# zeyadmohamedabdo/Visual-Question-Answering-VQA-system

Hardware: AMD Instinct MI355X
Metric: image-question pairs/sec (train step) (higher is better)
Workload: dtype bf16; 1 GPU; VQA train step fwd+CE+bwd+allreduce+clip+AdamW, batch 512/GPU, 3x224x224 images, 20 tokens, d=256, 4 text layers, 49 image tokens, 1000 answers, dropout on (BASELINE configs[2]); batch_per_gpu=512, global_batch=512, parallelism=dp1, reducer=off

## Files before the change

visual-question-answering-vqa-system_amd/csrc/cnn_ops.hip:

```cpp
#include "common.h"
#include "stem_route.h"

__global__ void bn_reduce_partials_kernel(const float* __restrict__ part, double* __restrict__ acc, int tiles, int C) {
  const int c = blockIdx.x * 64 + (threadIdx.x & 63), tl = threadIdx.x >> 6;
  __shared__ double sh[2][4][64];
  double s = 0.0, q = 0.0;
  if (c < C) {
    const int step = gridDim.y * 4;
    int t = blockIdx.y * 4 + tl;
    for (; t + 7 * step < tiles; t += 8 * step) {
      float a[8], b[8];
#pragma unroll
      for (int u = 0; u < 8; ++u) { a[u] = part[((size_t)(t + u * step) * 2) * C + c]; b[u] = part[((size_t)(t + u * step) * 2 + 1) * C + c]; }
#pragma unroll
      for (int u = 0; u < 8; ++u) { s += (double)a[u]; q += (double)b[u]; }
    }
    for (; t < tiles; t += step) {
      s += (double)part[((size_t)t * 2) * C + c];
      q += (double)part[((size_t)t * 2 + 1) * C + c];
    }
  }
  sh[0][tl][threadIdx.x & 63] = s; sh[1][tl][threadIdx.x & 63] = q;
  __syncthreads();
  if (tl == 0 && c < C) {
// ... 248 lines not shown
template <typename T, bool SELF, bool DUAL>
__global__ __launch_bounds__(256) void bn_bwd_apply_kernel(const T* __restrict__ dout, const T* __restrict__ outact, const T* __restrict__ y,
                                    const float* __restrict__ bc, T* __restrict__ dy, const T* __restrict__ y2,
                                    const float* __restrict__ bc2, T* __restrict__ dy2, size_t rows, int C,
                                    const float* __restrict__ mcoef) {
  constexpr int VEC = Vec16<T>::N;
  const int cv = C / VEC, lanes_r = 256 / cv;
  const int c0 = (threadIdx.x % cv) * VEC, myr = threadIdx.x / cv;
  float a[VEC], b[VEC], c[VEC], a2[DUAL ? VEC : 1], b2[DUAL ? VEC : 1], c2[DUAL ? VEC : 1], ms[SELF ? VEC : 1], mh[SELF ? VEC : 1];
#pragma unroll
  for (int j = 0; j < VEC; ++j) {
    a[j] = bc[c0 + j]; b[j] = bc[C + c0 + j]; c[j] = bc[2 * C + c0 + j];
    if (DUAL) { a2[j] = bc2[c0 + j]; b2[j] = bc2[C + c0 + j]; c2[j] = bc2[2 * C + c0 + j]; }
    if (SELF) { ms[j] = mcoef[c0 + j]; mh[j] = mcoef[C + c0 + j]; }
  }
#pragma unroll 2
  for (size_t r = (size_t)blockIdx.x * lanes_r + myr; r < rows; r += (size_t)gridDim.x * lanes_r) {
    const size_t off = r * C + c0;
    Vec16<T> d = ldg16(dout + off), yy = ldg16(y + off), o, y2v, rr, r2;
    if (!SELF && outact) o = ldg16(outact + off);
    if (DUAL) y2v = ldg16(y2 + off);
#pragma unroll
    for (int j = 0; j < VEC; ++j) {
      float g = d.get(j);
      if (SELF) { if (!(yy.get(j) * ms[j] + mh[j] > 0.f)) g = 0.f; }
      else if (outact && !(o.get(j) > 0.f)) g = 0.f;
      rr.set(j, a[j] * g + b[j] * yy.get(j) + c[j]);
      if (DUAL) r2.set(j, a2[j] * g + b2[j] * y2v.get(j) + c2[j]);
    }
    stg16(dy + off, rr);
    if (DUAL) stg16(dy2 + off, r2);
  }
}

template <typename T, bool SELF, bool DUAL>
__global__ __launch_bounds__(256) void bn_bwd_apply_acc_kernel(const T* __restrict__ dout, const T* __restrict__ outact, const T* __restrict__ y,
                                    const unsigned long long* __restrict__ facc, const float* __restrict__ gamma, const float* __restrict__ coef,
                                    float* dgamma, float* dbeta, T* __restrict__ dy, const T* __restrict__ y2, const float* __restrict__ gamma2,
                                    const float* __restrict__ coef2, float* dgamma2, float* dbeta2, T* __restrict__ dy2, size_t rows, int C,
                                    double inv_count) {
  constexpr int VEC = Vec16<T>::N;
  const int cv = C / VEC, lanes_r = 256 / cv;
  const int c0 = (threadIdx.x % cv) * VEC, myr = threadIdx.x / cv;
  const bool writer = blockIdx.x == 0;
  const int R = acc_replicas(C);
  const bool bad = acc_flagged(facc, R, 3, C);
  extern __shared__ float cf[];
  for (int ch = threadIdx.x; ch < C; ch += 256) {
    double sg = acc_read_fixed(facc, R, 3, C, 0, ch), sx = acc_read_fixed(facc, R, 3, C, 1, ch);
    if (bad) sg = sx = __builtin_nan("");
    const float mean = coef[2 * C + ch], invstd = coef[3 * C + ch], gi = gamma[ch] * invstd;
    const float mg = (float)(sg * inv_count), mgx = (float)(sx * inv_count);
    cf[ch] = gi; cf[C + ch] = -gi * invstd * mgx; cf[2 * C + ch] = gi * (mean * invstd * mgx - mg);
    if (writer) { dgamma[ch] += (float)sx; dbeta[ch] += (float)sg; }
    if (DUAL) {
      double sx2 = acc_read_fixed(facc, R, 3, C, 2, ch);
      if (bad) sx2 = __builtin_nan("");
      const float mean2 = coef2[2 * C + ch], inv2 = coef2[3 * C + ch], gi2 = gamma2[ch] * inv2, mgx2 = (float)(sx2 * inv_count);
      cf[3 * C + ch] = gi2; cf[4 * C + ch] = -gi2 * inv2 * mgx2; cf[5 * C + ch] = gi2 * (mean2 * inv2 * mgx2 - mg);
      if (writer) { dgamma2[ch] += (float)sx2; dbeta2[ch] += (float)sg; }
    }
  }
  __syncthreads();
  float a[VEC], b[VEC], c[VEC], a2[DUAL ? VEC : 1], b2[DUAL ? VEC : 1], c2[DUAL ? VEC : 1], ms[SELF ? VEC : 1], mh[SELF ? VEC : 1];
#pragma unroll
  for (int j = 0; j < VEC; ++j) {
    const int ch = c0 + j;
    a[j] = cf[ch]; b[j] = cf[C + ch]; c[j] = cf[2 * C + ch];
    if (DUAL) { a2[j] = cf[3 * C + ch]; b2[j] = cf[4 * C + ch]; c2[j] = cf[5 * C + ch]; }
    if (SELF) { ms[j] = coef[ch]; mh[j] = coef[C + ch]; }
  }
#pragma unroll 2
  for (size_t r = (size_t)blockIdx.x * lanes_r + myr; r < rows; r += (size_t)gridDim.x * lanes_r) {
    const size_t off = r * C + c0;
    Vec16<T> d = ldg16(dout + off), yy = ldg16(y + off), o, y2v, rr, r2;
    if (!SELF && outact) o = ldg16(outact + off);
    if (DUAL) y2v = ldg16(y2 + off);
#pragma unroll
    for (int j = 0; j < VEC; ++j) {
      float g = d.get(j);
      if (SELF) { if (!(yy.get(j) * ms[j] + mh[j] > 0.f)) g = 0.f; }
      else if (outact && !(o.get(j) > 0.f)) g = 0.f;
      rr.set(j, a[j] * g + b[j] * yy.get(j) + c[j]);
      if (DUAL) r2.set(j, a2[j] * g + b2[j] * y2v.get(j) + c2[j]);
    }
    stg16(dy + off, rr);
    if (DUAL) stg16(dy2 + off, r2);
  }
}

constexpr int SP_ROWS = 4, SP_PAIRS = 7;
template <typename T>
__global__ __launch_bounds__(256) void stem_pool_fwd_kernel(const T* __restrict__ y, const float* __restrict__ coef, T* __restrict__ out,
                                                            uint8_t* __restrict__ idx, int B, int H, int W, int C, int Ho, int Wo, int trows) {
  constexpr int VEC = Vec16<T>::N;
  const int cv = C / VEC, Wp = (Wo + 1) >> 1;
  const int tiles_x = (Wp + SP_PAIRS - 1) / SP_PAIRS, tiles_y = (Ho + trows - 1) / trows;
  const int per_row = SP_PAIRS * cv;
  const int ry = threadIdx.x / per_row, rem = threadIdx.x - ry * per_row;
  if (ry >= trows) return;
  const int pr = rem / cv, c0 = (rem - pr * cv) * VEC;
  int t = blockIdx.x;
  const int tx = t % tiles_x; t /= tiles_x; const int ty = t % tiles_y; const int b = t / tiles_y;
  const int oh = ty * trows + ry, owp = tx * SP_PAIRS + pr;
  if (oh >= Ho || owp >= Wp) return;
  float sc[VEC], sh[VEC];
#pragma unroll
  for (int j = 0; j < VEC; ++j) { sc[j] = coef[c0 + j]; sh[j] = coef[C + c0 + j]; }
  const int ow0 = owp * 2;
  const bool two = ow0 + 1 < Wo;
  float best[2][VEC]; int bi[2][VEC];
#pragma unroll
  for (int o = 0; o < 2; ++o)
#pragma unroll
    for (int j = 0; j < VEC; ++j) { best[o][j] = -INFINITY; bi[o][j] = 0; }
#pragma unroll
  for (int r = 0; r < 3; ++r) {
    const int ih = oh * 2 - 1 + r;
    if (ih < 0 || ih >= H) continue;
    const T* yr = y + (((size_t)b * H + ih) * W) * C + c0;
#pragma unroll
    for (int s5 = 0; s5 < 5; ++s5) {
      const int iw = ow0 * 2 - 1 + s5;
      if (iw < 0 || iw >= W) continue;
      const Vec16<T> yy = ldg16(yr + (size_t)iw * C);
      float a[VEC];
#pragma unroll
      for (int j = 0; j < VEC; ++j) { const float v = yy.get(j) * sc[j] + sh[j]; a[j] = v < 0.f ? 0.f : v; }
      if (s5 < 3) {
#pragma unroll
        for (int j = 0; j < VEC; ++j)
          if (a[j] > best[0][j] || a[j] != a[j]) { best[0][j] = a[j]; bi[0][j] = r * 3 + s5; }
      }
      if (s5 >= 2) {
#pragma unroll
        for (int j = 0; j < VEC; ++j)
          if (a[j] > best[1][j] || a[j] != a[j]) { best[1][j] = a[j]; bi[1][j] = r * 3 + s5 - 2; }
      }
    }
  }
#pragma unroll
  for (int o = 0; o < 2; ++o) {
    if (o == 1 && !two) break;
    const size_t e = ((((size_t)b * Ho + oh) * Wo + ow0 + o) * C + c0);
    Vec16<T> ov;
    uint32_t pk[VEC / 4];
#pragma unroll
    for (int q4 = 0; q4 < VEC / 4; ++q4) pk[q4] = 0u;
#pragma unroll
    for (int j = 0; j < VEC; ++j) { ov.set(j, best[o][j]); pk[j >> 2] |= (uint32_t)bi[o][j] << (8 * (j & 3)); }
    stg16(out + e, ov);
#pragma unroll
    for (int q4 = 0; q4 < VEC / 4; ++q4) reinterpret_cast<uint32_t*>(idx + e)[q4] = pk[q4];
  }
}

template <typename T>
__global__ void stem_bwd_apply_kernel(const T* __restrict__ dpool, const uint8_t* __restrict__ idx, const T* __restrict__ y,
                                      const float* __restrict__ coef, const float* __restrict__ bc, T* __restrict__ dy,
                                      int B, int H, int W, int C, int Ho, int Wo) {
  constexpr int VEC = Vec16<T>::N;
  const int cv = C / VEC;
  const size_t total = (size_t)B * H * W * cv;
  float g[VEC];
  for (size_t i = (size_t)blockIdx.x * blockDim.x + threadIdx.x; i < total; i += (size_t)gridDim.x * blockDim.x) {
    const int v = (int)(i % cv); size_t r = i / cv;
    const int w = (int)(r % W); size_t q = r / W; const int h = (int)(q % H); const int b = (int)(q / H);
    const int c0 = v * VEC;
    Vec16<T> yy = ldg16(y + i * VEC), o;
    float sc[VEC], sh[VEC];
#pragma unroll
    for (int j = 0; j < VEC; ++j) { sc[j] = coef[c0 + j]; sh[j] = coef[C + c0 + j]; }
    stem_route<T>(dpool, idx, yy, sc, sh, b, h, w, c0, C, Ho, Wo, g);
#pragma unroll
    for (int j = 0; j < VEC; ++j) o.set(j, bc[c0 + j] * g[j] + bc[C + c0 + j] * yy.get(j) + bc[2 * C + c0 + j]);
    stg16(dy + i * VEC, o);
  }
}

template <typename T>
__global__ __launch_bounds__(256) void se_pool_fc_kernel(const T* __restrict__ x, const float* __restrict__ w1, const float* __restrict__ w2,
                                                         float* __restrict__ pooled, float* __restrict__ hidden, float* __restrict__ scale,
                                                         int HW, int C, int Cr, const float* __restrict__ part, int chunks) {
  constexpr int VEC = Vec16<T>::N;
  extern __shared__ float sh[];
  const int b = blockIdx.x, cv = C / VEC, lanes_r = 256 / cv;
  const int myv = threadIdx.x % cv, myr = threadIdx.x / cv;
  float s[VEC];
#pragma unroll
  for (int j = 0; j < VEC; ++j) s[j] = 0.f;
  if (!part && myr < lanes_r) {
    const T* xb = x + (size_t)b * HW * C + myv * VEC;
    int p = myr;
    for (; p + 3 * lanes_r < HW; p += 4 * lanes_r) {
      Vec16<T> v0 = ldg16(xb + (size_t)p * C), v1 = ldg16(xb + (size_t)(p + lanes_r) * C);
      Vec16<T> v2 = ldg16(xb + (size_t)(p + 2 * lanes_r) * C), v3 = ldg16(xb + (size_t)(p + 3 * lanes_r) * C);
#pragma unroll
      for (int j = 0; j < VEC; ++j) s[j] += (v0.get(j) + v1.get(j)) + (v2.get(j) + v3.get(j));
    }
    for (; p < HW; p += lanes_r) {
      Vec16<T> v = ldg16(xb + (size_t)p * C);
#pragma unroll
      for (int j = 0; j < VEC; ++j) s[j] += v.get(j);
    }
  }
#pragma unroll
  for (int j = 0; j < VEC; ++j) sh[threadIdx.x * VEC + j] = s[j];
  __syncthreads();
  float* pl = sh + 256 * VEC; float* hd = pl + C;
  for (int c = threadIdx.x; c < C; c += 256) {
    const int v = c / VEC, j = c - v * VEC;
    float t = 0.f;
    if (part) { for (int k = 0; k < chunks; ++k) t += part[((size_t)b * chunks + k) * C + c]; }
    else { for (int r = 0; r < lanes_r; ++r) t += sh[(r * cv + v) * VEC + j]; }
    t /= (float)HW;
    pl[c] = t; pooled[(size_t)b * C + c] = t;
  }
  __syncthreads();
  const int lane = threadIdx.x & 63, wave = threadIdx.x >> 6;
  for (int jr = wave; jr < Cr; jr += 4) {
    float t = 0.f;
    for (int c = lane; c < C; c += 64) t += w1[(size_t)jr * C + c] * pl[c];
    t = wave_sum(t);
    if (lane == 0) { t = fmaxf(t, 0.f); hd[jr] = t; hidden[(size_t)b * Cr + jr] = t; }
  }
  __syncthreads();
  for (int c = threadIdx.x; c < C; c += 256) {
    float t = 0.f;
    for (int jr = 0; jr < Cr; ++jr) t += w2[(size_t)c * Cr + jr] * hd[jr];
    scale[(size_t)b * C + c] = 1.f / (1.f + expf(-t));
  }
}

template <typename T>
__global__ __launch_bounds__(256) void scale_kernel(const T* __restrict__ x, const float* __restrict__ chscale, const float* __restrict__ pixscale,
                                                    T* __restrict__ out, unsigned npix, int C, unsigned long long mul_hw) {
  constexpr int VEC = Vec16<T>::N;
  const int cv = C / VEC, lanes_r = 256 / cv, c0 = (threadIdx.x % cv) * VEC, myr = threadIdx.x / cv;
  for (unsigned pix = blockIdx.x * lanes_r + myr; pix < npix; pix += gridDim.x * lanes_r) {
    const size_t e = (size_t)pix * C + c0;
    Vec16<T> v = ldg16(x + e), o;
    const float ps = pixscale ? pixscale[pix] : 1.f;
    if (chscale) {
      const unsigned b = (unsigned)(((unsigned long long)pix * mul_hw) >> 40);
      const f32x4* cs = reinterpret_cast<const f32x4*>(chscale + (size_t)b * C + c0);
#pragma unroll
      for (int q4 = 0; q4 < VEC / 4; ++q4) {
        const f32x4 c4 = cs[q4];
#pragma unroll
        for (int j = 0; j < 4; ++j) o.set(q4 * 4 + j, v.get(q4 * 4 + j) * ps * c4[j]);
      }
    } else {
#pragma unroll
      for (int j = 0; j < VEC; ++j) o.set(j, v.get(j) * ps);
    }
    stg16(out + e, o);
  }
}

__device__ __forceinline__ void se_fc2_bwd(const float* __restrict__ z2, const float* __restrict__ w2, const float* __restrict__ hidden_b,
                                           float* __restrict__ dhs, float* __restrict__ dh_b, float* __restrict__ part, int C, int Cr, int NT) {
  if (Cr > NT) {
    for (int jr = threadIdx.x; jr < Cr; jr += NT) {
      float t = 0.f;
      for (int c = 0; c < C; ++c) t += z2[c] * w2[(size_t)c * Cr + jr];
      t = hidden_b[jr] > 0.f ? t : 0.f;
      dhs[jr] = t; dh_b[jr] = t;
    }
    __syncthreads();
    return;
  }
  const int G = min(NT / Cr, 64);
  const int jr = threadIdx.x % Cr, g = threadIdx.x / Cr;
  if (g < G) {
    float t = 0.f;
    for (int c = g; c < C; c += G) t += z2[c] * w2[(size_t)c * Cr + jr];
    part[g * Cr + jr] = t;
  }
  __syncthreads();
  if (threadIdx.x < Cr) {
    float t = 0.f;
    for (int q = 0; q < G; ++q) t += part[q * Cr + threadIdx.x];
    t = hidden_b[threadIdx.x] > 0.f ? t : 0.f;
    dhs[threadIdx.x] = t; dh_b[threadIdx.x] = t;
  }
  __syncthreads();
}

template <typename T>
__global__ __launch_bounds__(1024) void se_bwd_reduce_kernel(const T* __restrict__ dout, const T* __restrict__ x, const float* __restrict__ w1,
                                                            const float* __restrict__ w2, const float* __restrict__ hidden,
                                                            const float* __restrict__ scale, float* __restrict__ dz2, float* __restrict__ dh,
                                                            float* __restrict__ dpool, int HW, int C, int Cr) {
  constexpr int VEC = Vec16<T>::N;
  extern __shared__ float sh[];
  const int NT = blockDim.x;
  const int b = blockIdx.x, cv = C / VEC, lanes_r = NT / cv;
  const int myv = threadIdx.x % cv, myr = threadIdx.x / cv;
  float s[VEC];
#pragma unroll
  for (int j = 0; j < VEC; ++j) s[j] = 0.f;
  if (myr < lanes_r) {
    const size_t base = (size_t)b * HW * C + myv * VEC;
    int p = myr;
    for (; p + lanes_r < HW; p += 2 * lanes_r) {
      const size_t o0 = base + (size_t)p * C, o1 = base + (size_t)(p + lanes_r) * C;
// ... 461 lines not shown
  const size_t i = (size_t)blockIdx.x * blockDim.x + threadIdx.x;
  if (i >= (size_t)B * HW * C) return;
  const int c = (int)(i % C); size_t q = i / C; const int p = (int)(q % HW); const size_t b = q / HW;
  out[i] = from_f<T>(in[(b * C + c) * HW + p]);
}

static inline int px_grid(size_t npix, int C, int VEC) { const size_t lr = 256 / (C / VEC), g = (npix + lr - 1) / lr; return (int)(g > 16384 ? 16384 : (g ? g : 1)); }
static inline unsigned long long magic40(unsigned d) { return ((1ull << 40) + d - 1) / d; }
static inline int ew_grid(size_t n) { size_t g = (n + 255) / 256; return (int)(g > 16384 ? 16384 : (g ? g : 1)); }
static inline int row_grid(size_t rows, int lanes_r) { size_t g = (rows + lanes_r - 1) / lanes_r; return (int)(g > 8192 ? 8192 : (g ? g : 1)); }
#define DT(call_f, call_b) do { if (dtype) { call_b; } else { call_f; } } while (0)

extern "C" {

int vqa_bn_stats_finalize(const float* part, int tiles, int C, double count, const float* gamma, const float* beta,
                          float* running_mean, float* running_var, long long* nbt, float momentum, float eps,
                          double* scratch, float* coef, hipStream_t st) {
  if (!part || !scratch || !coef || tiles <= 0 || C <= 0) return VQA_EARG;
  int G = (tiles + 63) / 64; if (G > 64) G = 64; if (G < 1) G = 1;
  hipLaunchKernelGGL(bn_reduce_partials_kernel, dim3((C + 63) / 64, G), dim3(256), 0, st, part, scratch, tiles, C);
  hipLaunchKernelGGL(bn_finalize_kernel, dim3((C + 255) / 256), dim3(256), 0, st, scratch, G, C, count, gamma, beta,
                     running_mean, running_var, nbt, momentum, eps, coef);
  VQA_LAUNCH_CHECK(); return VQA_OK;
}
int vqa_bn_eval_coef(int C, const float* gamma, const float* beta, const float* rm, const float* rv, float eps, float* coef, hipStream_t st) {
  hipLaunchKernelGGL(bn_eval_coef_kernel, dim3((C + 255) / 256), dim3(256), 0, st, C, gamma, beta, rm, rv, eps, coef);
  VQA_LAUNCH_CHECK(); return VQA_OK;
}
int vqa_bn_apply(int dtype, const void* y, const float* coef, const void* res, const float* rcoef, void* out, long long numel, int C, int relu, hipStream_t st) {
  const int VEC = dtype ? 8 : 4;
  if (C % VEC || numel % C || C / VEC > 256 || 256 % (C / VEC)) return VQA_EARG;
  const size_t rows = (size_t)numel / C;
  const int grid = row_grid(rows, 256 / (C / VEC));
#define BN_APPLY(TT, R) hipLaunchKernelGGL((bn_apply_kernel<TT, R>), dim3(grid), dim3(256), 0, st, (const TT*)y, coef, (const TT*)res, rcoef, (TT*)out, rows, C, relu)
  const int mode = !res ? 0 : (rcoef ? 2 : 1);
  if (dtype) { if (mode == 0) BN_APPLY(bf16_t, 0); else if (mode == 1) BN_APPLY(bf16_t, 1); else BN_APPLY(bf16_t, 2); }
  else { if (mode == 0) BN_APPLY(float, 0); else if (mode == 1) BN_APPLY(float, 1); else BN_APPLY(float, 2); }
#undef BN_APPLY
  VQA_LAUNCH_CHECK(); return VQA_OK;
}
static inline int pool_rpc(int C, int VEC) { return (256 / (C / VEC)) * 14; }
int vqa_bn_apply_pool_chunks(int dtype, int HW, int C) {
  const int VEC = dtype ? 8 : 4;
  if (C % VEC || C / VEC > 256 || 256 % (C / VEC) || HW <= 0) return 0;
  return (HW + pool_rpc(C, VEC) - 1) / pool_rpc(C, VEC);
}
int vqa_bn_apply_pool(int dtype, const void* y, const float* coef, const void* res, const float* rcoef, void* out, int B, int HW, int C,
                      int relu, float* part, hipStream_t st) {
  const int VEC = dtype ? 8 : 4;
  const int chunks = vqa_bn_apply_pool_chunks(dtype, HW, C);
  if (!y || !coef || !out || !part || B <= 0 || chunks <= 0 || B > 65535) return VQA_EARG;
  const int rpc = pool_rpc(C, VEC);
#define BN_APPLYP(TT, R) hipLaunchKernelGGL((bn_apply_pool_kernel<TT, R>), dim3(chunks, B), dim3(256), 0, st, (const TT*)y, coef, (const TT*)res, rcoef, (TT*)out, HW, C, relu, rpc, part)
  const int mode = !res ? 0 : (rcoef ? 2 : 1);
  if (dtype) { if (mode == 0) BN_APPLYP(bf16_t, 0); else if (mode == 1) BN_APPLYP(bf16_t, 1); else BN_APPLYP(bf16_t, 2); }
  else { if (mode == 0) BN_APPLYP(float, 0); else if (mode == 1) BN_APPLYP(float, 1); else BN_APPLYP(float, 2); }
#undef BN_APPLYP
  VQA_LAUNCH_CHECK(); return VQA_OK;
}
int vqa_bn_acc_words(int K, int C) { const long long w = 2ll * acc_replicas(C) * K * C + 1; return (int)((w + 1) / 2 * 2); }
int vqa_bn_apply_acc(int dtype, const void* y, const unsigned long long* acc, const float* gamma, const float* beta, float* rm, float* rv,
                     long long* nbt, float* coef_out, const void* res, const unsigned long long* racc, const float* rgamma, const float* rbeta,
                     float* rrm, float* rrv, long long* rnbt, float* rcoef_out, void* out, int B, int HW, int C, int relu, double count,
                     float momentum, float eps, float* pool_part, hipStream_t st) {
  const int VEC = dtype ? 8 : 4;
  if (!y || !acc || !gamma || !beta || !coef_out || !out || B <= 0 || HW <= 0 || C % VEC || C / VEC > 256 || 256 % (C / VEC)) return VQA_EARG;
  if (racc && (!res || !rgamma || !rbeta || !rcoef_out)) return VQA_EARG;
  if (pool_part && racc) return VQA_EARG;
  BnAcc f = {acc, gamma, beta, rm, rv, nbt, coef_out}, fr = {racc, rgamma, rbeta, rrm, rrv, rnbt, rcoef_out};
  const size_t rows = (size_t)B * HW;
  const int lanes_r = 256 / (C / VEC);
  int g1 = row_grid(rows, lanes_r);
  { const int cap = vqa_env_int("VQA_BN_GRID", res ? 512 : 1024); if (g1 > cap) g1 = cap; }
  dim3 grid(g1);
  int rpc = 0;
  const double inv_count = 1.0 / count, unbias = count > 1.0 ? count / (count - 1.0) : 1.0;
  const size_t shm = (size_t)(racc ? 4 : 2) * C * sizeof(float);
  if (pool_part) {
    const int chunks = vqa_bn_apply_pool_chunks(dtype, HW, C);
    if (chunks <= 0 || B > 65535) return VQA_EARG;
    rpc = pool_rpc(C, VEC); grid = dim3(chunks, B);
  }
#define BN_ACC(TT, R, PL) hipLaunchKernelGGL((bn_apply_acc_kernel<TT, R, PL>), grid, dim3(256), shm, st, (const TT*)y, f, (const TT*)res, fr, (TT*)out, rows, HW, C, \
    relu, rpc, inv_count, unbias, momentum, eps, pool_part)
  const int mode = !res ? 0 : (racc ? 2 : 1);
  if (dtype) {
    if (pool_part) { if (mode == 0) BN_ACC(bf16_t, 0, true); else BN_ACC(bf16_t, 1, true); }
    else { if (mode == 0) BN_ACC(bf16_t, 0, false); else if (mode == 1) BN_ACC(bf16_t, 1, false); else BN_ACC(bf16_t, 2, false); }
  } else {
    if (pool_part) { if (mode == 0) BN_ACC(float, 0, true); else BN_ACC(float, 1, true); }
    else { if (mode == 0) BN_ACC(float, 0, false); else if (mode == 1) BN_ACC(float, 1, false); else BN_ACC(float, 2, false); }
  }
#undef BN_ACC
  VQA_LAUNCH_CHECK(); return VQA_OK;
}
int vqa_bn_bwd_blocks(long long rows) { long long g = (rows + 63) / 64; const int cap = vqa_env_int("VQA_BNR_GRID", rows < 65536 ? 256 : 512); return (int)(g > cap ? cap : (g < 1 ? 1 : g)); }
int vqa_bn_bwd_reduce(int dtype, const void* dout, const void* outact, const void* y, const float* coef, const void* y2, const float* coef2,
                      float* slab, long long rows, int C, int self_mask, int acc_mode, hipStream_t st) {
  const int VEC = dtype ? 8 : 4;
  if (C % VEC || C / VEC > 256 || 256 % (C / VEC)) return VQA_EARG;
  const int nb = vqa_bn_bwd_blocks(rows);
  const size_t shm = (size_t)3 * 256 * VEC * 4;
#define BWD_RED(TT, S, D) hipLaunchKernelGGL((bn_bwd_reduce_kernel<TT, S, D>), dim3(nb), dim3(256), shm, st, (const TT*)dout, (const TT*)outact, \
    (const TT*)y, coef, (const TT*)y2, coef2, acc_mode ? nullptr : slab, (size_t)rows, C, acc_mode ? (unsigned long long*)slab : nullptr)
  if (self_mask && (y2 || outact)) return VQA_EARG;
  if (dtype) { if (self_mask) BWD_RED(bf16_t, true, false); else if (y2) BWD_RED(bf16_t, false, true); else BWD_RED(bf16_t, false, false); }
  else { if (self_mask) BWD_RED(float, true, false); else if (y2) BWD_RED(float, false, true); else BWD_RED(float, false, false); }
#undef BWD_RED
  VQA_LAUNCH_CHECK(); return VQA_OK;
}
int vqa_bn_bwd_finalize(const float* slab, int nblk, int C, int which, double count, const float* gamma, const float* coef, int training,
                        float* dgamma, float* dbeta, float* bcoef, hipStream_t st) {
  hipLaunchKernelGGL(bn_bwd_finalize_kernel, dim3((C + 63) / 64), dim3(1024), 0, st, slab, nblk, C, which, count, gamma, coef, training, dgamma, dbeta, bcoef);
  VQA_LAUNCH_CHECK(); return VQA_OK;
}
int vqa_bn_bwd_apply_acc(int dtype, const void* dout, const void* outact, const void* y, const unsigned long long* facc, const float* gamma,
                         const float* coef, float* dgamma, float* dbeta, void* dy, const void* y2, const float* gamma2, const float* coef2,
                         float* dgamma2, float* dbeta2, void* dy2, long long numel, int C, double count, int self_mask, hipStream_t st) {
  const int VEC = dtype ? 8 : 4;
  if (!dout || !y || !facc || !gamma || !coef || !dgamma || !dbeta || !dy || C % VEC || numel % C || C / VEC > 256 || 256 % (C / VEC)) return VQA_EARG;
  if (y2 && (!gamma2 || !coef2 || !dgamma2 || !dbeta2 || !dy2)) return VQA_EARG;
  if (self_mask && (y2 || outact)) return VQA_EARG;
  const size_t rows = (size_t)numel / C;
  int grid = row_grid(rows, 256 / (C / VEC));
  { const int cap = vqa_env_int("VQA_BNB_GRID", 512); if (grid > cap) grid = cap; }
  const size_t shm = (size_t)(y2 ? 6 : 3) * C * sizeof(float);
  const double inv_count = 1.0 / count;
#define BWD_ACC(TT, S, D) hipLaunchKernelGGL((bn_bwd_apply_acc_kernel<TT, S, D>), dim3(grid), dim3(256), shm, st, (const TT*)dout, (const TT*)outact, \
    (const TT*)y, facc, gamma, coef, dgamma, dbeta, (TT*)dy, (const TT*)y2, gamma2, coef2, dgamma2, dbeta2, (TT*)dy2, rows, C, inv_count)
  if (dtype) { if (self_mask) BWD_ACC(bf16_t, true, false); else if (y2) BWD_ACC(bf16_t, false, true); else BWD_ACC(bf16_t, false, false); }
  else { if (self_mask) BWD_ACC(float, true, false); else if (y2) BWD_ACC(float, false, true); else BWD_ACC(float, false, false); }
#undef BWD_ACC
  VQA_LAUNCH_CHECK(); return VQA_OK;
}
int vqa_bn_bwd_apply(int dtype, const void* dout, const void* outact, const void* y, const float* bc, void* dy,
                     const void* y2, const float* bc2, void* dy2, long long numel, int C, const float* mask_coef, hipStream_t st) {
  const int VEC = dtype ? 8 : 4;
  if (C % VEC || numel % C || C / VEC > 256 || 256 % (C / VEC)) return VQA_EARG;
  const size_t rows = (size_t)numel / C;
  const int grid = row_grid(rows, 256 / (C / VEC));
#define BWD_APPLY(TT, S, D) hipLaunchKernelGGL((bn_bwd_apply_kernel<TT, S, D>), dim3(grid), dim3(256), 0, st, (const TT*)dout, (const TT*)outact, \
    (const TT*)y, bc, (TT*)dy, (const TT*)y2, bc2, (TT*)dy2, rows, C, mask_coef)
  if (mask_coef && (y2 || outact)) return VQA_EARG;
  if (dtype) { if (mask_coef) BWD_APPLY(bf16_t, true, false); else if (y2) BWD_APPLY(bf16_t, false, true); else BWD_APPLY(bf16_t, false, false); }
  else { if (mask_coef) BWD_APPLY(float, true, false); else if (y2) BWD_APPLY(float, false, true); else BWD_APPLY(float, false, false); }
#undef BWD_APPLY
  VQA_LAUNCH_CHECK(); return VQA_OK;
}

int vqa_stem_pool_fwd(int dtype, const void* y, const float* coef, void* out, uint8_t* idx, int B, int H, int W, int C, hipStream_t st) {
  const int VEC = dtype ? 8 : 4, Ho = (H + 2 - 3) / 2 + 1, Wo = (W + 2 - 3) / 2 + 1;
  const int per_row = SP_PAIRS * (C / VEC);
  if (C % 8 || per_row > 256) return VQA_EARG;
  const int trows = 256 / per_row < SP_ROWS ? 256 / per_row : SP_ROWS;
  const int Wp = (Wo + 1) / 2;
  const long long tiles = (long long)B * ((Ho + trows - 1) / trows) * ((Wp + SP_PAIRS - 1) / SP_PAIRS);
  if (tiles <= 0 || tiles > 0x7fffffffll) return VQA_EARG;
  const int threads = (per_row * trows + 63) / 64 * 64;
  DT(hipLaunchKernelGGL(stem_pool_fwd_kernel<float>, dim3((unsigned)tiles), dim3(threads), 0, st, (const float*)y, coef, (float*)out, idx, B, H, W, C, Ho, Wo, trows),
     hipLaunchKernelGGL(stem_pool_fwd_kernel<bf16_t>, dim3((unsigned)tiles), dim3(threads), 0, st, (const bf16_t*)y, coef, (bf16_t*)out, idx, B, H, W, C, Ho, Wo, trows));
  VQA_LAUNCH_CHECK(); return VQA_OK;
}
int vqa_stem_bwd_apply(int dtype, const void* dpool, const uint8_t* idx, const void* y, const float* coef, const float* bc, void* dy, int B, int H, int W, int C, hipStream_t st) {
  const int VEC = dtype ? 8 : 4, Ho = (H + 2 - 3) / 2 + 1, Wo = (W + 2 - 3) / 2 + 1;
  const size_t total = (size_t)B * H * W * (C / VEC);
  DT(hipLaunchKernelGGL(stem_bwd_apply_kernel<float>, dim3(ew_grid(total)), dim3(256), 0, st, (const float*)dpool, idx, (const float*)y, coef, bc, (float*)dy, B, H, W, C, Ho, Wo),
     hipLaunchKernelGGL(stem_bwd_apply_kernel<bf16_t>, dim3(ew_grid(total)), dim3(256), 0, st, (const bf16_t*)dpool, idx, (const bf16_t*)y, coef, bc, (bf16_t*)dy, B, H, W, C, Ho, Wo));
  VQA_LAUNCH_CHECK(); return VQA_OK;
}

int vqa_se_fwd(int dtype, const void* x, const float* w1, const float* w2, float* pooled, float* hidden, float* scale, void* out,
               int B, int HW, int C, int Cr, const float* pool_part, int pool_chunks, hipStream_t st) {
  const int VEC = dtype ? 8 : 4;
  if (C % VEC || C / VEC > 256 || 256 % (C / VEC) || Cr < 1 || Cr > C) return VQA_EARG;
  if (pool_part && pool_chunks != vqa_bn_apply_pool_chunks(dtype, HW, C)) return VQA_EARG;
  const size_t shm = ((size_t)256 * VEC + C + Cr) * 4;
  DT(hipLaunchKernelGGL(se_pool_fc_kernel<float>, dim3(B), dim3(256), shm, st, (const float*)x, w1, w2, pooled, hidden, scale, HW, C, Cr, pool_part, pool_chunks),
     hipLaunchKernelGGL(se_pool_fc_kernel<bf16_t>, dim3(B), dim3(256), shm, st, (const bf16_t*)x, w1, w2, pooled, hidden, scale, HW, C, Cr, pool_part, pool_chunks));
  const size_t npix = (size_t)B * HW;
  if (npix >= (1ull << 28)) return VQA_EARG;
  DT(hipLaunchKernelGGL(scale_kernel<float>, dim3(px_grid(npix, C, VEC)), dim3(256), 0, st, (const float*)x, scale, (const float*)nullptr, (float*)out, (unsigned)npix, C, magic40(HW)),
     hipLaunchKernelGGL(scale_kernel<bf16_t>, dim3(px_grid(npix, C, VEC)), dim3(256), 0, st, (const bf16_t*)x, scale, (const float*)nullptr, (bf16_t*)out, (unsigned)npix, C, magic40(HW)));
  VQA_LAUNCH_CHECK(); return VQA_OK;
}
int vqa_se_bwd_blocks(int dtype, int B, int HW, int C) {
  const int VEC = dtype ? 8 : 4;
  if (C % VEC || C / VEC > 256 || 256 % (C / VEC)) return 0;
  const int g = px_grid((size_t)B * HW, C, VEC);
  return g > 2048 ? 2048 : g;
}
static bool se_bwd_nreg_off() { return vqa_env_int("VQA_SE_NREG", 1) == 0; }
static bool se_bwd_nlds_off() { return vqa_env_int("VQA_SE_NLDS", 1) == 0; }
long long vqa_se_bwd_scratch(int dtype, int B, int HW, int C, int Cr) { (void)dtype; (void)HW; return (long long)B * (2 * C + Cr); }
int vqa_se_bwd(int dtype, const void* dout, const void* x, const float* w1, const float* w2, const float* pooled, const float* hidden,
               const float* scale, float* scratch, void* dx, float* dw1, float* dw2, int B, int HW, int C, int Cr, int mask_out,
               const void* bn_y, const float* bn_coef, float* bn_slab, int bn_acc_mode, hipStream_t st) {
  const int VEC = dtype ? 8 : 4;
  if (C % VEC || C / VEC > 256 || 256 % (C / VEC) || Cr < 1 || Cr > C) return VQA_EARG;
  if ((bn_slab != nullptr) != (bn_y != nullptr) || (bn_slab != nullptr) != (bn_coef != nullptr)) return VQA_EARG;
  if ((dw1 != nullptr) != (dw2 != nullptr)) return VQA_EARG;
  float* dz2 = scratch; float* dh = dz2 + (size_t)B * C; float* dpool = dh + (size_t)B * Cr;
  const int cvh = C / VEC;
  const int nt = (1024 % cvh == 0 && (long long)HW * cvh >= (dtype ? 2048 : 4096)) ? 1024 : 256;
  const size_t shm = ((size_t)nt * VEC + C + Cr) * 4;
  const bool accm = (bn_acc_mode & 1) != 0;
  if (bn_slab && accm && B > VQA_ACC_MAX_PARTS) return VQA_EARG;
  if (!bn_slab || accm) {
    const size_t shm2 = ((size_t)nt * VEC + 3 * C + Cr) * 4;
#define SE_FUSED(TT, R) hipLaunchKernelGGL((se_bwd_fused_kernel<TT, R>), dim3(B), dim3(nt), shm2, st, (const TT*)dout, (const TT*)x, w1, w2, hidden, scale, \
    dz2, dh, dpool, (TT*)dx, HW, C, Cr, mask_out, (const TT*)bn_y, bn_coef, (unsigned long long*)bn_slab)
#define SE_FUSED_K(R_, NR, NL) do { if (tailm) SE_FUSED_KT(R_, NR, NL, true); else SE_FUSED_KT(R_, NR, NL, false); } while (0)
#define SE_FUSED_KT(R_, NR, NL, TM) do { \
      const size_t shl = ((shm2 + 15) & ~(size_t)15) + (size_t)(NL) * nt * 17 + ((TM) ? (size_t)ntail * nt : 0); \
      auto kfn = se_bwd_fused_kernel<bf16_t, R_, NR, NL, TM>; \
      (void)vqa_ensure_lds(reinterpret_cast<const void*>(kfn), shl); \
      hipLaunchKernelGGL(kfn, dim3(B), dim3(nt), shl, st, (const bf16_t*)dout, (const bf16_t*)x, w1, w2, hidden, scale, dz2, dh, dpool, (bf16_t*)dx, \
                         HW, C, Cr, mask_out, (const bf16_t*)bn_y, bn_coef, (unsigned long long*)bn_slab); } while (0)
#define SE_FUSED_D(R_) do { if (nreg == 2) SE_FUSED_K(R_, 2, 0); else if (nlds == 0) SE_FUSED_K(R_, 4, 0); else if (nlds == 2) SE_FUSED_K(R_, 4, 2); \
      else if (nlds == 4) SE_FUSED_K(R_, 4, 4); else SE_FUSED_K(R_, 4, 6); } while (0)
    const int nit = (HW + nt / cvh - 1) / (nt / cvh);
    const int nreg = !dtype || se_bwd_nreg_off() ? 0 : nit <= 2 ? 2 : 4;
    int nlds = (nreg == 4 && nt == 1024 && !se_bwd_nlds_off()) ? (nit <= 4 ? 0 : nit <= 6 ? 2 : nit <= 8 ? 4 : 6) : 0;
    while (nlds > 0 && ((shm2 + 15) & ~(size_t)15) + (size_t)nlds * nt * 17 > 160 * 1024) nlds -= 2;
    const int ntail = nit - nreg - nlds > 0 ? nit - nreg - nlds : 0;
    const bool tailm = nreg == 4 && mask_out && ntail > 0 && !se_bwd_nlds_off() &&
                       ((shm2 + 15) & ~(size_t)15) + (size_t)nlds * nt * 17 + (size_t)ntail * nt <= 156 * 1024;
    if (dtype && nreg) { if (bn_slab) SE_FUSED_D(true); else SE_FUSED_D(false); }
    else if (dtype) { if (bn_slab) SE_FUSED(bf16_t, true); else SE_FUSED(bf16_t, false); }
    else { if (bn_slab) SE_FUSED(float, true); else SE_FUSED(float, false); }
#undef SE_FUSED_K
#undef SE_FUSED_KT
#undef SE_FUSED_D
#undef SE_FUSED
    if (dw1) launch_se_wgrad(dz2, hidden, dh, pooled, dw1, dw2, B, C, Cr, st);
    VQA_LAUNCH_CHECK(); return VQA_OK;
  }
  DT(hipLaunchKernelGGL(se_bwd_reduce_kernel<float>, dim3(B), dim3(nt), shm, st, (const float*)dout, (const float*)x, w1, w2, hidden, scale, dz2, dh, dpool, HW, C, Cr),
     hipLaunchKernelGGL(se_bwd_reduce_kernel<bf16_t>, dim3(B), dim3(nt), shm, st, (const bf16_t*)dout, (const bf16_t*)x, w1, w2, hidden, scale, dz2, dh, dpool, HW, C, Cr));
  const size_t npix = (size_t)B * HW;
  if (npix >= (1ull << 28)) return VQA_EARG;
  const int ag = bn_slab ? vqa_se_bwd_blocks(dtype, B, HW, C) : px_grid(npix, C, VEC);
#define SE_APPLY(TT, R) hipLaunchKernelGGL((se_bwd_apply_kernel<TT, R>), dim3(ag), dim3(256), 0, st, (const TT*)dout, scale, dpool, (TT*)dx, (unsigned)npix, HW, C, \
    magic40(HW), mask_out ? (const TT*)x : nullptr, (const TT*)bn_y, bn_coef, accm ? nullptr : bn_slab, \
    accm ? (unsigned long long*)bn_slab : nullptr)
  if (dtype) { if (bn_slab) SE_APPLY(bf16_t, true); else SE_APPLY(bf16_t, false); }
  else { if (bn_slab) SE_APPLY(float, true); else SE_APPLY(float, false); }
#undef SE_APPLY
  if (dw1) launch_se_wgrad(dz2, hidden, dh, pooled, dw1, dw2, B, C, Cr, st);
  VQA_LAUNCH_CHECK(); return VQA_OK;
}

int vqa_spatial_fwd(int dtype, const void* x, const float* w, float* pooled2, int* amax, float* amap, void* out, int B, int H, int W, int C, hipStream_t st) {
  const int VEC = dtype ? 8 : 4;
  const size_t npix = (size_t)B * H * W;
  if (C <= 0 || C % VEC || npix >= (1ull << 28) || C / VEC > 256 || 256 % (C / VEC)) return VQA_EARG;
  const int pg = (int)((npix + 3) / 4 > 8192 ? 8192 : (npix + 3) / 4);
  DT(hipLaunchKernelGGL(spatial_pool_kernel<float>, dim3(pg), dim3(256), 0, st, (const float*)x, pooled2, amax, npix, C),
     hipLaunchKernelGGL(spatial_pool_kernel<bf16_t>, dim3(pg), dim3(256), 0, st, (const bf16_t*)x, pooled2, amax, npix, C));
  hipLaunchKernelGGL(spatial_conv_kernel, dim3((unsigned)((npix + 255) / 256)), dim3(256), 0, st, pooled2, w, amap, B, H, W);
  DT(hipLaunchKernelGGL(scale_kernel<float>, dim3(px_grid(npix, C, VEC)), dim3(256), 0, st, (const float*)x, (const float*)nullptr, amap, (float*)out, (unsigned)npix, C, magic40(H * W)),
     hipLaunchKernelGGL(scale_kernel<bf16_t>, dim3(px_grid(npix, C, VEC)), dim3(256), 0, st, (const bf16_t*)x, (const float*)nullptr, amap, (bf16_t*)out, (unsigned)npix, C, magic40(H * W)));
  VQA_LAUNCH_CHECK(); return VQA_OK;
}
long long vqa_spatial_bwd_scratch(int B, int H, int W) { return 3ll * B * H * W + SPATIAL_WG_SLICES * 98; }
int vqa_spatial_bwd(int dtype, const void* dout, const void* x, const float* w, const float* pooled2, const int* amax, const float* amap,
                    float* scratch, void* dx, float* dw, int B, int H, int W, int C, hipStream_t st) {
  const int VEC = dtype ? 8 : 4;
  const size_t npix = (size_t)B * H * W;
  if (C <= 0 || C % VEC || npix >= (1ull << 28) || C / VEC > 256 || 256 % (C / VEC)) return VQA_EARG;
  float* dpre = scratch; float* dpool2 = dpre + npix; float* wpart = dpool2 + 2 * npix;
  const int pg = (int)((npix + 3) / 4 > 8192 ? 8192 : (npix + 3) / 4);
  DT(hipLaunchKernelGGL(spatial_bwd_reduce_kernel<float>, dim3(pg), dim3(256), 0, st, (const float*)dout, (const float*)x, amap, dpre, npix, C),
     hipLaunchKernelGGL(spatial_bwd_reduce_kernel<bf16_t>, dim3(pg), dim3(256), 0, st, (const bf16_t*)dout, (const bf16_t*)x, amap, dpre, npix, C));
  hipLaunchKernelGGL(spatial_bwd_conv_kernel, dim3((unsigned)((npix + 255) / 256)), dim3(256), 0, st, dpre, w, dpool2, B, H, W);
  DT(hipLaunchKernelGGL(spatial_bwd_apply_kernel<float>, dim3(px_grid(npix, C, VEC)), dim3(256), 0, st, (const float*)dout, amap, dpool2, amax, (float*)dx, (unsigned)npix, C),
     hipLaunchKernelGGL(spatial_bwd_apply_kernel<bf16_t>, dim3(px_grid(npix, C, VEC)), dim3(256), 0, st, (const bf16_t*)dout, amap, dpool2, amax, (bf16_t*)dx, (unsigned)npix, C));
  if (dw) {
    hipLaunchKernelGGL(spatial_wgrad_kernel, dim3(98, SPATIAL_WG_SLICES), dim3(256), 0, st, dpre, pooled2, wpart, B, H, W);
    hipLaunchKernelGGL(spatial_wgrad_finish_kernel, dim3(1), dim3(128), 0, st, wpart, dw);
  }
  VQA_LAUNCH_CHECK(); return VQA_OK;
}

int vqa_nhwc_to_nchw(int dtype, const void* in, float* out, int B, int HW, int C, hipStream_t st) {
  const size_t n = (size_t)B * HW * C;
  DT(hipLaunchKernelGGL(nhwc_to_nchw_kernel<float>, dim3((unsigned)((n + 255) / 256)), dim3(256), 0, st, (const float*)in, out, B, HW, C),
     hipLaunchKernelGGL(nhwc_to_nchw_kernel<bf16_t>, dim3((unsigned)((n + 255) / 256)), dim3(256), 0, st, (const bf16_t*)in, out, B, HW, C));
  VQA_LAUNCH_CHECK(); return VQA_OK;
}
int vqa_nchw_to_nhwc(int dtype, const float* in, void* out, int B, int HW, int C, hipStream_t st) {
  const size_t n = (size_t)B * HW * C;
  DT(hipLaunchKernelGGL(nchw_to_nhwc_kernel<float>, dim3((unsigned)((n + 255) / 256)), dim3(256), 0, st, in, (float*)out, B, HW, C),
     hipLaunchKernelGGL(nchw_to_nhwc_kernel<bf16_t>, dim3((unsigned)((n + 255) / 256)), dim3(256), 0, st, in, (bf16_t*)out, B, HW, C));
  VQA_LAUNCH_CHECK(); return VQA_OK;
}

}
```

Measured before the change: 42050 pairs/s.

## Add banded row-streaming bf16 stem BN+ReLU+maxpool forward kernel with carried row reuse

```diff
diff --git a/visual-question-answering-vqa-system_amd/csrc/cnn_ops.hip b/visual-question-answering-vqa-system_amd/csrc/cnn_ops.hip
--- a/visual-question-answering-vqa-system_amd/csrc/cnn_ops.hip
+++ b/visual-question-answering-vqa-system_amd/csrc/cnn_ops.hip
@@ -424,6 +424,97 @@
     stg16(out + e, ov);
 #pragma unroll
     for (int q4 = 0; q4 < VEC / 4; ++q4) reinterpret_cast<uint32_t*>(idx + e)[q4] = pk[q4];
+  }
+}
+
+constexpr int SPS_BAND = 14, SPS_BAND_MIN = 5;
+typedef __attribute__((ext_vector_type(2))) float sps_f2;
+struct SpsRow { float m[8]; uint32_t s[8]; };
+__device__ __forceinline__ float sps_max3(float a, float b, float c) { return __builtin_elementwise_maximum(__builtin_elementwise_maximum(a, b), c); }
+__device__ __forceinline__ bool sps_any_nan(const float (&m)[8]) {
+  return (m[0] != m[0]) | (m[1] != m[1]) | (m[2] != m[2]) | (m[3] != m[3]) | (m[4] != m[4]) | (m[5] != m[5]) | (m[6] != m[6]) | (m[7] != m[7]);
+}
+__device__ __forceinline__ void sps_load(const bf16_t* __restrict__ yb, int ih, int H, size_t rstride, const int (&coff)[3], Vec16<bf16_t> (&v)[3]) {
+  const bf16_t* yr = yb + (size_t)min(max(ih, 0), H - 1) * rstride;
+#pragma unroll
+  for (int s = 0; s < 3; ++s) v[s] = ldg16(yr + coff[s]);
+}
+__device__ __forceinline__ void sps_bn(const Vec16<bf16_t>& v, const sps_f2 (&sc)[4], const sps_f2 (&sh)[4], float (&a)[8]) {
+#pragma unroll
+  for (int i = 0; i < 4; ++i) {
+    const uint32_t w = v.raw[i];
+    const sps_f2 x = {__uint_as_float(w << 16), __uint_as_float(w & 0xffff0000u)};
+    const sps_f2 r = x * sc[i] + sh[i];
+    a[2 * i] = r.x; a[2 * i + 1] = r.y;
+  }
+}
+__device__ __forceinline__ void sps_reduce(const Vec16<bf16_t> (&v)[3], uint32_t code0, uint32_t base, bool ok2, const sps_f2 (&sc)[4], const sps_f2 (&sh)[4], SpsRow& o) {
+  float a0[8], a1[8], a2[8];
+  sps_bn(v[0], sc, sh, a0); sps_bn(v[1], sc, sh, a1); sps_bn(v[2], sc, sh, a2);
+#pragma unroll
+  for (int j = 0; j < 8; ++j) {
+    o.m[j] = sps_max3(a0[j], a1[j], a2[j]);
+    o.s[j] = a0[j] == o.m[j] ? code0 : (a1[j] == o.m[j] ? base + 1u : base + 2u);
+  }
+  if (sps_any_nan(o.m)) {
+#pragma unroll
+    for (int j = 0; j < 8; ++j)
+      if (o.m[j] != o.m[j]) o.s[j] = (ok2 && a2[j] != a2[j]) ? base + 2u : (a1[j] != a1[j] ? base + 1u : code0);
+  }
+}
+__global__ __launch_bounds__(256) void stem_pool_rows_kernel(const bf16_t* __restrict__ y, const float* __restrict__ coef, bf16_t* __restrict__ out,
+                                                             uint8_t* __restrict__ idx, int H, int W, int C, int Ho, int Wo, int band, int nbands, int nchunks) {
+  const int cv = C >> 3;
+  int t = blockIdx.x;
+  const int chunk = t % nchunks; t /= nchunks; const int bd = t % nbands; const int b = t / nbands;
+  const int item = chunk * 256 + threadIdx.x;
+  if (item >= Wo * cv) return;
+  const int ow = item / cv, c0 = (item - ow * cv) * 8;
+  sps_f2 sc[4], sh[4];
+#pragma unroll
+  for (int i = 0; i < 4; ++i) { sc[i] = sps_f2{coef[c0 + 2 * i], coef[c0 + 2 * i + 1]}; sh[i] = sps_f2{coef[C + c0 + 2 * i], coef[C + c0 + 2 * i + 1]}; }
+  const uint32_t left = ow > 0 ? 0u : 1u;
+  const bool ok2 = 2 * ow + 1 < W;
+  const int coff[3] = {max(2 * ow - 1, 0) * C, 2 * ow * C, min(2 * ow + 1, W - 1) * C};
+  const size_t rstride = (size_t)W * C;
+  const bf16_t* yb = y + (size_t)b * H * rstride + c0;
+  const int oh0 = bd * band, oh1 = min(Ho, oh0 + band);
+  SpsRow car;
+  {
+    Vec16<bf16_t> v[3];
+    sps_load(yb, 2 * oh0 - 1, H, rstride, coff, v);
+    sps_reduce(v, oh0 > 0 ? left : 3u + left, oh0 > 0 ? 0u : 3u, ok2, sc, sh, car);
+  }
+  size_t e = ((((size_t)b * Ho + oh0) * Wo + ow) * C + c0);
+  for (int oh = oh0; oh < oh1; ++oh, e += (size_t)Wo * C) {
+    Vec16<bf16_t> va[3], vb[3];
+    sps_load(yb, 2 * oh, H, rstride, coff, va);
+    sps_load(yb, 2 * oh + 1, H, rstride, coff, vb);
+    SpsRow ra, rb;
+    sps_reduce(va, 3u + left, 3u, ok2, sc, sh, ra);
+    sps_reduce(vb, left, 0u, ok2, sc, sh, rb);
+    const uint32_t zc = (oh > 0 ? 0u : 3u) + left;
+    float M[8]; uint32_t code[8];
+#pragma unroll
+    for (int j = 0; j < 8; ++j) {
+      M[j] = sps_max3(car.m[j], ra.m[j], rb.m[j]);
+      const uint32_t kc = car.m[j] == M[j] ? car.s[j] : 15u, ka = ra.m[j] == M[j] ? ra.s[j] : 15u;
+      code[j] = min(min(kc, ka), rb.s[j] + 6u);
+      code[j] = M[j] <= 0.f ? zc : code[j];
+    }
+    if (sps_any_nan(M)) {
+      const bool bok = 2 * oh + 1 < H;
+#pragma unroll
+      for (int j = 0; j < 8; ++j)
+        if (M[j] != M[j]) code[j] = (bok && rb.m[j] != rb.m[j]) ? rb.s[j] + 6u : (ra.m[j] != ra.m[j] ? ra.s[j] : car.s[j]);
+    }
+    Vec16<bf16_t> ov;
+    uint32_t pk[2] = {0u, 0u};
+#pragma unroll
+    for (int j = 0; j < 8; ++j) { ov.set(j, M[j] < 0.f ? 0.f : M[j]); pk[j >> 2] |= code[j] << (8 * (j & 3)); }
+    stg16(out + e, ov);
+    *reinterpret_cast<uint2*>(idx + e) = make_uint2(pk[0], pk[1]);
+    car = rb;
   }
 }
 
@@ -1191,6 +1282,18 @@
   const int VEC = dtype ? 8 : 4, Ho = (H + 2 - 3) / 2 + 1, Wo = (W + 2 - 3) / 2 + 1;
   const int per_row = SP_PAIRS * (C / VEC);
   if (C % 8 || per_row > 256) return VQA_EARG;
+  if (dtype) {
+    if (!y || !coef || !out || !idx || B <= 0 || H <= 0 || W <= 0) return VQA_EARG;
+    const int nchunks = (Wo * (C / 8) + 255) / 256;
+    int band = vqa_env_int("VQA_SPOOL_BAND", SPS_BAND);
+    if (band < 1) band = 1;
+    while (band > SPS_BAND_MIN && (long long)B * ((Ho + band - 1) / band) * nchunks < 512) band = band / 2 > SPS_BAND_MIN ? band / 2 : SPS_BAND_MIN;
+    const int nbands = (Ho + band - 1) / band;
+    const long long wgs = (long long)B * nbands * nchunks;
+    if (wgs > 0x7fffffffll) return VQA_EARG;
+    hipLaunchKernelGGL(stem_pool_rows_kernel, dim3((unsigned)wgs), dim3(256), 0, st, (const bf16_t*)y, coef, (bf16_t*)out, idx, H, W, C, Ho, Wo, band, nbands, nchunks);
+    VQA_LAUNCH_CHECK(); return VQA_OK;
+  }
   const int trows = 256 / per_row < SP_ROWS ? 256 / per_row : SP_ROWS;
   const int Wp = (Wo + 1) / 2;
   const long long tiles = (long long)B * ((Ho + trows - 1) / trows) * ((Wp + SP_PAIRS - 1) / SP_PAIRS);
```

Measured after the change: 42240 pairs/s, median of 6. About the same (+0.5%).
